# lachinov/brats2019

Hardware: AMD Instinct MI355X
Metric: volumes_per_sec_fwd_bwd_128cubed_x4ch (higher is better)
Workload: dtype bf16

## Files before the change

### brats2019_amd/csrc/pointwise_c16.hip

```cpp
#include "pw_helpers.hpp"
#include "fin_tail.hpp"
#include <type_traits>
#include <stdlib.h>

namespace ru {

typedef float f32x4_c16 __attribute__((ext_vector_type(4)));
template <int I, int N, class F> __device__ __forceinline__ void static_for_c1_impl(F&& f) {
    if constexpr (I < N) { f(std::integral_constant<int, I>{}); static_for_c1_impl<I + 1, N>(f); }
}
template <int N, class F> __device__ __forceinline__ void static_for_c1(F&& f) { static_for_c1_impl<0, N>(f); }

static inline dim3 c16_grid(size_t V, int blocks_nc, unsigned cap = 2048) {
    size_t bx = (V * 4 + 255) / 256;
    if (bx > cap) bx = cap;
    if (bx < 1) bx = 1;
    return dim3((unsigned)bx, (unsigned)blocks_nc);
}

template <int RES, bool NT = false>
__global__ __launch_bounds__(256) void gn_apply16_kernel(const float* __restrict__ x, const float* __restrict__ scale, const float* __restrict__ shift,
                                                         const float* __restrict__ res, float* __restrict__ y, int C, size_t V, float slope,
                                                         const float* __restrict__ rscale, const float* __restrict__ rshift, float rslope) {
    const int nb = blockIdx.y, CB = C >> 4;
// ... 101 lines not shown
    const int nblk = gn_bwd_tiles16(V);
    FinTail f{};
    if (fin) f = *fin;
    RU_REQUIRE(!f.ticket || (f.kind == 2 && f.nblk == nblk && f.N == N && f.C == C && f.G == G), "gn_bwd_reduce16: tail descriptor does not match the launch");
    const size_t lds = 512 + fin_tail_lds_bytes(f);
    RU_REQUIRE(lds <= 64 * 1024, "gn_bwd_reduce16: batch x channels too large for the in-launch finalize");
    hipLaunchKernelGGL(gn_bwd_reduce16_kernel, dim3(nblk, N * (C / 16)), dim3(256), lds, s, x, dy, scale, shift, mean, rstd, slope, partials, C, V, G, nblk, gn16_chunk(V), f);
    RU_CHECK_LAUNCH("gn_bwd_reduce16_kernel");
    return RU_OK;
}

__global__ __launch_bounds__(256) void gn_bwd_apply16_kernel(const float* __restrict__ x, const float* __restrict__ dy, const float* __restrict__ scale,
                                                             const float* __restrict__ shift, const float* __restrict__ coef, float slope,
                                                             float* __restrict__ dx, int C, size_t V) {
    const int nb = blockIdx.y, CB = C >> 4;
    const int n = nb / CB, cb = nb - n * CB;
    const int q = threadIdx.x & 3;
    const size_t row = (size_t)n * C + cb * 16 + 4 * q;
    float a[4], b[4], cA[4], cB[4], cC[4];
#pragma unroll
    for (int k = 0; k < 4; ++k) {
        a[k] = scale[row + k]; b[k] = shift[row + k];
        cA[k] = coef[(row + k) * 3]; cB[k] = coef[(row + k) * 3 + 1]; cC[k] = coef[(row + k) * 3 + 2];
    }
    const size_t base = (size_t)nb * V * 4, F = V * 4;
    const float4* xp = reinterpret_cast<const float4*>(x) + base;
    const float4* dp = reinterpret_cast<const float4*>(dy) + base;
    float4* op = reinterpret_cast<float4*>(dx) + base;
    for (size_t f = (size_t)blockIdx.x * 256 + threadIdx.x; f < F; f += (size_t)gridDim.x * 256) {
        const float4 t = xp[f], d = dp[f];
        float4 o;
        o.x = cA[0] * ((t.x * a[0] + b[0]) > 0.f ? d.x : d.x * slope) + (cB[0] * t.x + cC[0]);
        o.y = cA[1] * ((t.y * a[1] + b[1]) > 0.f ? d.y : d.y * slope) + (cB[1] * t.y + cC[1]);
        o.z = cA[2] * ((t.z * a[2] + b[2]) > 0.f ? d.z : d.z * slope) + (cB[2] * t.z + cC[2]);
        o.w = cA[3] * ((t.w * a[3] + b[3]) > 0.f ? d.w : d.w * slope) + (cB[3] * t.w + cC[3]);
        op[f] = o;
    }
}
__global__ __launch_bounds__(256) void gn_bwd_apply16_split_kernel(const float* __restrict__ x, const float* __restrict__ dy, const float* __restrict__ scale,
                                                                   const float* __restrict__ shift, const float* __restrict__ coef, float slope,
                                                                   float* __restrict__ dx, int C, size_t V) {
    const int nb = blockIdx.y, CB = C >> 4;
    const int n = nb / CB, cb = nb - n * CB;
    const int hf = threadIdx.x & 1;
    const size_t row = (size_t)n * C + cb * 16 + 8 * hf;
    float a[8], b[8], cA[8], cB[8], cC[8];
#pragma unroll
    for (int k = 0; k < 8; ++k) {
        a[k] = scale[row + k]; b[k] = shift[row + k];
        cA[k] = coef[(row + k) * 3]; cB[k] = coef[(row + k) * 3 + 1]; cC[k] = coef[(row + k) * 3 + 2];
    }
    const size_t base = (size_t)nb * V * 4, F = V * 2;
    const float4* xp = reinterpret_cast<const float4*>(x) + base;
    const float4* dp = reinterpret_cast<const float4*>(dy) + base;
    pw_u32x4* op = reinterpret_cast<pw_u32x4*>(dx) + base;
    for (size_t f = (size_t)blockIdx.x * 256 + threadIdx.x; f < F; f += (size_t)gridDim.x * 256) {
        const size_t v = f >> 1;
        const float4 t0 = xp[v * 4 + 2 * hf], t1 = xp[v * 4 + 2 * hf + 1], d0 = dp[v * 4 + 2 * hf], d1 = dp[v * 4 + 2 * hf + 1];
        const float tx[8] = {t0.x, t0.y, t0.z, t0.w, t1.x, t1.y, t1.z, t1.w}, dd[8] = {d0.x, d0.y, d0.z, d0.w, d1.x, d1.y, d1.z, d1.w};
        float o[8];
#pragma unroll
        for (int k = 0; k < 8; ++k) o[k] = cA[k] * ((tx[k] * a[k] + b[k]) > 0.f ? dd[k] : dd[k] * slope) + (cB[k] * tx[k] + cC[k]);
        pw_u32x4 hi, lo;
        pw_split8(o, hi, lo);
        op[v * 4 + hf] = hi;
        op[v * 4 + 2 + hf] = lo;
    }
}
int gn_bwd_apply16_launch(const float* x, const float* dy, const float* scale, const float* shift, const float* coef, float slope, float* dx,
                          int N, int C, size_t V, int split, hipStream_t s) {
    RU_REQUIRE(C % 16 == 0, "gn_bwd_apply16: C must be a multiple of 16");
    if (split) {
        size_t bx = (V * 2 + 255) / 256;
        if (bx > 2048) bx = 2048;
        hipLaunchKernelGGL(gn_bwd_apply16_split_kernel, dim3((unsigned)bx, (unsigned)(N * (C / 16))), dim3(256), 0, s, x, dy, scale, shift, coef, slope, dx, C, V);
    } else {
        hipLaunchKernelGGL(gn_bwd_apply16_kernel, c16_grid(V, N * (C / 16)), dim3(256), 0, s, x, dy, scale, shift, coef, slope, dx, C, V);
    }
    RU_CHECK_LAUNCH("gn_bwd_apply16_kernel");
    return RU_OK;
}

__global__ __launch_bounds__(256) void up2_fwd16_kernel(const float* __restrict__ x, float* __restrict__ y, int D, int H, int W, float slope) {
    const int Do = 2 * D, Ho = 2 * H, Wo = 2 * W;
    const size_t nb = blockIdx.y;
    const size_t Vi = (size_t)D * H * W, Vo = Vi * 8;
    const float4* xp = reinterpret_cast<const float4*>(x) + nb * Vi * 4;
    float4* yp = reinterpret_cast<float4*>(y) + nb * Vo * 4;
    const bool nt_out = (size_t)gridDim.y * Vo * 16 * sizeof(float) >= ((size_t)128 << 20);
    const size_t total = (size_t)(D + 1) * (H + 1) * Wo * 4;
    for (size_t f = (size_t)blockIdx.x * 256 + threadIdx.x; f < total; f += (size_t)gridDim.x * 256) {
        const int q = (int)(f & 3);
        size_t r = f >> 2;
        const int xo = (int)(r % Wo); r /= Wo;
        const int ky = (int)(r % (H + 1)) - 1;
        const int kz = (int)(r / (H + 1)) - 1;
        int x0, x1; float lx0, lx1;
        up2_src(xo, W, x0, x1, lx0, lx1);
        const int zA = kz < 0 ? 0 : kz, zB = kz + 1 > D - 1 ? D - 1 : kz + 1;
        const int yA = ky < 0 ? 0 : ky, yB = ky + 1 > H - 1 ? H - 1 : ky + 1;
        const size_t rAA = ((size_t)zA * H + yA) * W, rAB = ((size_t)zA * H + yB) * W, rBA = ((size_t)zB * H + yA) * W, rBB = ((size_t)zB * H + yB) * W;
        const float4 a00 = xp[(rAA + x0) * 4 + q], b00 = xp[(rAA + x1) * 4 + q];
        const float4 a01 = xp[(rAB + x0) * 4 + q], b01 = xp[(rAB + x1) * 4 + q];
        const float4 a10 = xp[(rBA + x0) * 4 + q], b10 = xp[(rBA + x1) * 4 + q];
        const float4 a11 = xp[(rBB + x0) * 4 + q], b11 = xp[(rBB + x1) * 4 + q];
        float4 e00, e01, e10, e11;
#define RU_UPX(c) e00.c = lx0 * a00.c + lx1 * b00.c; e01.c = lx0 * a01.c + lx1 * b01.c; e10.c = lx0 * a10.c + lx1 * b10.c; e11.c = lx0 * a11.c + lx1 * b11.c
        RU_UPX(x); RU_UPX(y); RU_UPX(z); RU_UPX(w);
#undef RU_UPX
#pragma unroll
        for (int dz = 0; dz < 2; ++dz) {
            const int zo = 2 * kz + 1 + dz;
            if (zo < 0 || zo >= Do) continue;
            int z0, z1; float lz0, lz1;
            up2_src(zo, D, z0, z1, lz0, lz1);
#pragma unroll
            for (int dy = 0; dy < 2; ++dy) {
                const int yo = 2 * ky + 1 + dy;
                if (yo < 0 || yo >= Ho) continue;
                int y0, y1; float ly0, ly1;
                up2_src(yo, H, y0, y1, ly0, ly1);
                float4 o;
#define RU_UP2(c) o.c = lrelu(lz0 * (ly0 * e00.c + ly1 * e01.c) + lz1 * (ly0 * e10.c + ly1 * e11.c), slope)
                RU_UP2(x); RU_UP2(y); RU_UP2(z); RU_UP2(w);
#undef RU_UP2
                if (nt_out) __builtin_nontemporal_store(f32x4_c16{o.x, o.y, o.z, o.w}, reinterpret_cast<f32x4_c16*>(yp + (((size_t)zo * Ho + yo) * Wo + xo) * 4 + q));
                else yp[(((size_t)zo * Ho + yo) * Wo + xo) * 4 + q] = o;
            }
        }
    }
}
int up2_fwd16_launch(const float* x, float* y, int N, int C, int D, int H, int W, float slope, hipStream_t s) {
    RU_REQUIRE(C % 16 == 0, "up2_fwd16: C must be a multiple of 16");
    const size_t total = (size_t)(D + 1) * (H + 1) * (2 * W) * 4;
    size_t bx = (total + 255) / 256;
    if (bx > 16384) bx = 16384;
    hipLaunchKernelGGL(up2_fwd16_kernel, dim3((unsigned)bx, (unsigned)(N * (C / 16))), dim3(256), 0, s, x, y, D, H, W, slope);
    RU_CHECK_LAUNCH("up2_fwd16_kernel");
    return RU_OK;
}

#ifndef RU_UP2B_ZC
#define RU_UP2B_ZC 8
#endif
constexpr int UP2B_ZC = RU_UP2B_ZC;
__global__ __launch_bounds__(256) void up2_bwd16_kernel(const float* __restrict__ dy, float* __restrict__ dx, int D, int H, int W) {
    const int Do = 2 * D, Ho = 2 * H, Wo = 2 * W;
    const size_t nb = blockIdx.y;
    const size_t Vi = (size_t)D * H * W, Vo = Vi * 8;
    const float4* dp = reinterpret_cast<const float4*>(dy) + nb * Vo * 4;
    float4* op = reinterpret_cast<float4*>(dx) + nb * Vi * 4;
    const int nch = (D + UP2B_ZC - 1) / UP2B_ZC;
    const size_t total = (size_t)nch * H * W * 4;
    for (size_t f = (size_t)blockIdx.x * 256 + threadIdx.x; f < total; f += (size_t)gridDim.x * 256) {
        const int q = (int)(f & 3);
        size_t r = f >> 2;
        const int kx = (int)(r % W); r /= W;
        const int ky = (int)(r % H);
        const int k0 = (int)(r / H) * UP2B_ZC;
        const int k1 = k0 + UP2B_ZC < D ? k0 + UP2B_ZC : D;
        float wy[4], wx[4];
        size_t oy[4], ox[4];
#pragma unroll
        for (int t = 0; t < 4; ++t) {
            const int y = 2 * ky - 1 + t, xx = 2 * kx - 1 + t;
            wy[t] = (y >= 0 && y < Ho) ? up2_coef(y, H, ky) : 0.f;
            wx[t] = (xx >= 0 && xx < Wo) ? up2_coef(xx, W, kx) : 0.f;
            oy[t] = (size_t)(y < 0 ? 0 : (y >= Ho ? Ho - 1 : y)) * Wo;
            ox[t] = (size_t)(xx < 0 ? 0 : (xx >= Wo ? Wo - 1 : xx)) * 4 + q;
        }
        float4 accP = make_float4(0.f, 0.f, 0.f, 0.f), accC = accP;
        for (int m = k0; m <= k1; ++m) {
#pragma unroll
            for (int h = 0; h < 2; ++h) {
                const int z = 2 * m - 1 + h;
                const bool in = z >= 0 && z < Do;
                const size_t zrow = (size_t)(z < 0 ? 0 : (z >= Do ? Do - 1 : z)) * Ho * Wo;
                float4 pz = make_float4(0.f, 0.f, 0.f, 0.f);
#pragma unroll
                for (int b = 0; b < 4; ++b) {
                    const float4* row = dp + (zrow + oy[b]) * 4;
                    const float4 p0 = row[ox[0]], p1 = row[ox[1]], p2 = row[ox[2]], p3 = row[ox[3]];
                    pz.x += wy[b] * (wx[0] * p0.x + wx[1] * p1.x + wx[2] * p2.x + wx[3] * p3.x);
                    pz.y += wy[b] * (wx[0] * p0.y + wx[1] * p1.y + wx[2] * p2.y + wx[3] * p3.y);
                    pz.z += wy[b] * (wx[0] * p0.z + wx[1] * p1.z + wx[2] * p2.z + wx[3] * p3.z);
                    pz.w += wy[b] * (wx[0] * p0.w + wx[1] * p1.w + wx[2] * p2.w + wx[3] * p3.w);
                }
                const float cP = (in && m - 1 >= k0) ? up2_coef(z, D, m - 1) : 0.f;
                const float cC = (in && m < k1) ? up2_coef(z, D, m) : 0.f;
                accP.x += cP * pz.x; accP.y += cP * pz.y; accP.z += cP * pz.z; accP.w += cP * pz.w;
                accC.x += cC * pz.x; accC.y += cC * pz.y; accC.z += cC * pz.z; accC.w += cC * pz.w;
            }
            if (m - 1 >= k0) op[(((size_t)(m - 1) * H + ky) * W + kx) * 4 + q] = accP;
            accP = accC;
            accC = make_float4(0.f, 0.f, 0.f, 0.f);
        }
    }
}
int up2_bwd16_launch(const float* dy, float* dx, int N, int C, int D, int H, int W, hipStream_t s) {
    RU_REQUIRE(C % 16 == 0, "up2_bwd16: C must be a multiple of 16");
    const size_t total = (size_t)((D + UP2B_ZC - 1) / UP2B_ZC) * H * W * 4;
    size_t bx = (total + 255) / 256;
    if (bx > 16384) bx = 16384;
    hipLaunchKernelGGL(up2_bwd16_kernel, dim3((unsigned)bx, (unsigned)(N * (C / 16))), dim3(256), 0, s, dy, dx, D, H, W);
    RU_CHECK_LAUNCH("up2_bwd16_kernel");
    return RU_OK;
}

__global__ void pack_down16_kernel(const float* __restrict__ w, float* __restrict__ wd, float* __restrict__ wdT, int Cout, int Cin) {
    const int i = blockIdx.x * blockDim.x + threadIdx.x;
    if (i >= Cout * Cin * 8) return;
    const int tap = i & 7, c = (i >> 3) % Cin, o = i / (8 * Cin);
    const float v = w[i];
    wd[(size_t)o * 8 * Cin + tap * Cin + c] = v;
    wdT[(size_t)(tap * Cin + c) * Cout + o] = v;
}
int pack_down16_launch(const float* w, float* wd, float* wdT, int Cout, int Cin, hipStream_t s) {
    const int total = Cout * Cin * 8;
    hipLaunchKernelGGL(pack_down16_kernel, dim3(cdiv(total, 256)), dim3(256), 0, s, w, wd, wdT, Cout, Cin);
    RU_CHECK_LAUNCH("pack_down16_kernel");
    return RU_OK;
}

template <int COB, int S2D, int NSLOT, bool PAIR = false>
__global__ __launch_bounds__(256, (PAIR || NSLOT > 0) ? 2 : 1) void conv1_16_kernel(const Conv1Args a, int nvt) {
    static_assert(!PAIR || (S2D == 2 && COB == 4 && (NSLOT == 1 || NSLOT == 2)), "paired stores: the scatter mode with statistics, four blocks per workgroup");
    constexpr bool BST = NSLOT > 0;
    constexpr int NSL = BST ? NSLOT : 1;
    __shared__ float red[BST ? 4 * NSL * 16 * 2 : 1];
    const int lane = threadIdx.x & 63, wave = threadIdx.x >> 6;
    const int n = blockIdx.z, cog = blockIdx.y;
    const size_t V = a.V;
    const int r = lane & 15, g = lane >> 4;
    const int nkb0 = a.C0 >> 4, nkb1 = a.C1 >> 4, nkb = nkb0 + nkb1, CBo = a.Cout >> 4;
    const int Hf = 2 * a.Hc, Wf = 2 * a.Wc;
    const size_t Vf = V * 8;
    const int CBf_out = CBo >> 3;
    const int Cstat = S2D == 2 ? (a.Cout >> 3) : a.Cout;
    f32x4_c16 bs1[NSL], bs2[NSL], bk[NSL][3];
    if constexpr (BST) {
#pragma unroll
        for (int sl = 0; sl < NSL; ++sl) {
            bs1[sl] = f32x4_c16{0.f, 0.f, 0.f, 0.f}; bs2[sl] = f32x4_c16{0.f, 0.f, 0.f, 0.f};
            const int cob = cog * COB + sl, chb = S2D == 2 ? cob % CBf_out : cob;
            const float* kp = a.bst_k + (size_t)n * 3 * Cstat + (cob < CBo ? chb : 0) * 16 + 4 * g;
#pragma unroll
            for (int t3 = 0; t3 < 3; ++t3) { const float4 q = *reinterpret_cast<const float4*>(kp + (size_t)t3 * Cstat); bk[sl][t3] = f32x4_c16{q.x, q.y, q.z, q.w}; }
        }
    }
    const bool nt_out = (size_t)a.N * a.Cout * V * sizeof(float) >= ((size_t)128 << 20);
    const int vt = blockIdx.x * 4 + wave;
    const bool live = vt < nvt;
    if (!live) { if constexpr (!BST) return; }
    if (live) {
    const size_t v0 = (size_t)vt * 64;
    size_t vb[4], fv[4];
#pragma unroll
    for (int t = 0; t < 4; ++t) {
        size_t v = v0 + 16 * t + r;
        if (v >= V) v = V - 1;
        vb[t] = v * 16 + 4 * g;
        fv[t] = 0;
        if constexpr (S2D != 0) {
            const int xc = (int)(v % a.Wc);
            const size_t rr = v / a.Wc;
            const int yc = (int)(rr % a.Hc), zc = (int)(rr / a.Hc);
            fv[t] = ((size_t)(2 * zc) * Hf + 2 * yc) * Wf + 2 * xc;
        }
    }
    const float* wrow[COB];
#pragma unroll
    for (int cb = 0; cb < COB; ++cb) {
        const int cob = cog * COB + cb;
        wrow[cb] = a.wT + (size_t)((cob < CBo ? cob : CBo - 1) * 16 + r) * a.ldw + 4 * g;
    }
    f32x4_c16 acc[4][COB];
#pragma unroll
    for (int t = 0; t < 4; ++t)
#pragma unroll
        for (int cb = 0; cb < COB; ++cb) acc[t][cb] = f32x4_c16{0.f, 0.f, 0.f, 0.f};
    const int CBf_in = nkb0 >> 3;
    auto kstep = [&](int kb) __attribute__((always_inline)) {
        float4 xb[4];
        if constexpr (S2D == 1) {
            const int tap = kb / CBf_in, cbf = kb - tap * CBf_in;
            const size_t toff = ((size_t)(tap >> 2) * Hf + ((tap >> 1) & 1)) * Wf + (tap & 1);
            const float* src = a.x0 + ((size_t)(n * CBf_in + cbf) * Vf) * 16 + 4 * g;
#pragma unroll
            for (int t = 0; t < 4; ++t) xb[t] = *reinterpret_cast<const float4*>(src + (fv[t] + toff) * 16);
        } else {
            const float* src = kb < nkb0 ? a.x0 + ((size_t)(n * nkb0 + kb) * V) * 16 : a.x1 + ((size_t)(n * nkb1 + kb - nkb0) * V) * 16;
#pragma unroll
            for (int t = 0; t < 4; ++t) xb[t] = *reinterpret_cast<const float4*>(src + vb[t]);
        }
#pragma unroll
        for (int cb = 0; cb < COB; ++cb) {
            const float4 wv = *reinterpret_cast<const float4*>(wrow[cb] + kb * 16);
#pragma unroll
            for (int t = 0; t < 4; ++t) {
                acc[t][cb] = __builtin_amdgcn_mfma_f32_16x16x4f32(wv.x, xb[t].x, acc[t][cb], 0, 0, 0);
                acc[t][cb] = __builtin_amdgcn_mfma_f32_16x16x4f32(wv.y, xb[t].y, acc[t][cb], 0, 0, 0);
                acc[t][cb] = __builtin_amdgcn_mfma_f32_16x16x4f32(wv.z, xb[t].z, acc[t][cb], 0, 0, 0);
                acc[t][cb] = __builtin_amdgcn_mfma_f32_16x16x4f32(wv.w, xb[t].w, acc[t][cb], 0, 0, 0);
            }
        }
    };
    int kb = 0;
// ... 290 lines not shown
```

### brats2019_amd/csrc/wgrad_tr.hip

```cpp
#include "ru_common.h"

#include <utility>

namespace ru {

typedef float f32x4 __attribute__((ext_vector_type(4)));
typedef __bf16 bf16x8 __attribute__((ext_vector_type(8)));
typedef __bf16 bf16x2 __attribute__((ext_vector_type(2)));
typedef short s16x4 __attribute__((ext_vector_type(4)));
typedef short s16x8 __attribute__((ext_vector_type(8)));
typedef unsigned int u32x4 __attribute__((ext_vector_type(4)));


template <int... Is, class F>
__device__ __forceinline__ void wt_static_for_impl(std::integer_sequence<int, Is...>, F&& f) {
    (f(std::integral_constant<int, Is>{}), ...);
}
template <int N, class F>
__device__ __forceinline__ void wt_static_for(F&& f) {
    wt_static_for_impl(std::make_integer_sequence<int, N>{}, static_cast<F&&>(f));
}

__device__ __forceinline__ void wt_split8(const float (&t)[8], u32x4& hi, u32x4& lo) {
    split_n<4>(t, hi, lo);
}

__device__ __forceinline__ void wt_hi8(const float (&t)[8], u32x4& hi) {
#pragma unroll
    for (int i = 0; i < 4; ++i) {
        ru_bf16x2 h;
        h[0] = (__bf16)t[2 * i];
        h[1] = (__bf16)t[2 * i + 1];
        hi[i] = __builtin_bit_cast(unsigned, h);
    }
}

__device__ __forceinline__ bf16x8 wt_read_tr(const char* p0, const char* p1) {
    const s16x4 a = __builtin_amdgcn_ds_read_tr16_b64_v4i16((s16x4 __attribute__((address_space(3)))*)(p0));
    const s16x4 b = __builtin_amdgcn_ds_read_tr16_b64_v4i16((s16x4 __attribute__((address_space(3)))*)(p1));
    const s16x8 r = {a[0], a[1], a[2], a[3], b[0], b[1], b[2], b[3]};
    return __builtin_bit_cast(bf16x8, r);
}

template <int OT>
struct WTZ {
    static constexpr int TY = 8, HY = 10, HX = 18, NSLOT = 8;
    static constexpr int PPOS = HY * HX;
    static constexpr int PLANE = PPOS * 32;
    static constexpr int XRING = NSLOT * PLANE;
    static constexpr int X_OFF = 0, XLO_OFF = XRING;
    static constexpr int DPOS = 2 * TY * 16, DPLANE = DPOS * 32;
    static constexpr int DBUF = OT * 2 * DPLANE;
    static constexpr int D_OFF = 2 * XRING;
    static constexpr int LDS = 2 * XRING + 2 * DBUF;
    static constexpr int NKB = 8;
};

template <int OT, int NP, bool PACK>
__device__ __forceinline__ void wtz_consume(const char* __restrict__ xl, const int (&pw)[3], const char* __restrict__ dl, f32x4 (&acc)[27]) {
    using P = WTZ<OT>;
    constexpr int HX = P::HX, NHALF = OT, NG = PACK ? 3 : 9, NU = NHALF * NG;
    bf16x8 bh[2][4], bl[2][4];
    bf16x8 ah[2][2], al[2][2];
    auto read_one = [&](auto U, auto R) {
        constexpr int u = decltype(U)::value, r = NP == 3 ? decltype(R)::value : 2 * decltype(R)::value;
        constexpr int h = u / NG, g = u % NG, dz = PACK ? g : g / 3, dx = PACK ? 0 : g % 3, set = u & 1;
        if constexpr (r < 8) {
            constexpr int pr = r >> 1;
            constexpr int off0 = ((4 * h + pr) * HX + dx) * 32, off1 = off0 + 2 * HX * 32;
            const char* p = xl + pw[dz];
            if constexpr ((r & 1) == 0) bh[set][pr] = wt_read_tr(p + P::X_OFF + off0, p + P::X_OFF + off1);
            else bl[set][pr] = wt_read_tr(p + P::XLO_OFF + off0, p + P::XLO_OFF + off1);
        } else {
            constexpr int ra = r - 8, kbi = ra >> 1;
            constexpr int off0 = (4 * h + kbi) * 16 * 32, off1 = off0 + 2 * 16 * 32;
            if constexpr ((ra & 1) == 0) ah[h & 1][kbi] = wt_read_tr(dl + off0, dl + off1);
            else al[h & 1][kbi] = wt_read_tr(dl + P::DPLANE + off0, dl + P::DPLANE + off1);
        }
    };
    auto nreads = [](int u) constexpr { return ((u % NG == 0) ? 12 : 8) / (NP == 3 ? 1 : 2); };
    wt_static_for<nreads(0)>([&](auto R) { read_one(std::integral_constant<int, 0>{}, R); });
    wt_static_for<NU>([&](auto U) {
        constexpr int u = decltype(U)::value, h = u / NG, g = u % NG, dz = PACK ? g : g / 3, dx = PACK ? 0 : g % 3, set = u & 1;
        constexpr int nr = u + 1 < NU ? nreads(u + 1) : 0;
        constexpr int NM = 6 * NP;
        wt_static_for<NM>([&](auto M) {
            constexpr int m = decltype(M)::value, prod = NP == 3 ? m / 6 : 2, kbi = (m / 3) % 2, dy = m % 3;
            constexpr int tap = PACK ? dz * 3 + dy : dz * 9 + dy * 3 + dx, pr = kbi + dy;
            if constexpr (prod == 0) acc[tap] = __builtin_amdgcn_mfma_f32_16x16x32_bf16(al[h & 1][kbi], bh[set][pr], acc[tap], 0, 0, 0);
            if constexpr (prod == 1) acc[tap] = __builtin_amdgcn_mfma_f32_16x16x32_bf16(ah[h & 1][kbi], bl[set][pr], acc[tap], 0, 0, 0);
            if constexpr (prod == 2) acc[tap] = __builtin_amdgcn_mfma_f32_16x16x32_bf16(ah[h & 1][kbi], bh[set][pr], acc[tap], 0, 0, 0);
            __builtin_amdgcn_sched_barrier(0);
            constexpr int ra = m * nr / NM, rb = (m + 1) * nr / NM;
            wt_static_for<rb - ra>([&](auto K) {
                read_one(std::integral_constant<int, u + 1>{}, std::integral_constant<int, ra + decltype(K)::value>{});
            });
            __builtin_amdgcn_sched_barrier(0);
        });
    });
}

template <int OT, int XS, int DS, int NP = 3>
__global__ __launch_bounds__(512, 2) void wgrad3_tz_kernel(const Wgrad3Args a, float* __restrict__ partials, int ntz, int nty, int ntx, int ncg, int CoP, int CiP) {
    using P = WTZ<OT>;
    constexpr int HX = P::HX, PPOS = P::PPOS, DPOS = P::DPOS, TY = P::TY;
    constexpr bool FA = DS == 3 || DS == 4, G16 = DS == 4;
    extern __shared__ __attribute__((aligned(256))) char lds[];

    const int tid = threadIdx.x, lane = tid & 63;
    const int wave = __builtin_amdgcn_readfirstlane(tid >> 6);
    const bool producer = wave >= 4;
    const int rw = wave & 3, ptid = tid & 255;
    const int og = blockIdx.y / ncg, cgp = blockIdx.y % ncg;
    const int D = a.D, H = a.H, W = a.W;
    const size_t DHW = (size_t)D * H * W;
    const int CBi = a.Cin >> 4, CBo = a.Cout >> 4;
    const int cols_per_sample = nty * ntx, ncol = a.N * cols_per_sample;
    const int G = gridDim.x;
    const int swz = (G % 8 == 0) ? (blockIdx.x % 8) * (G / 8) + blockIdx.x / 8 : blockIdx.x;
    const int mycols = swz < ncol ? (ncol - swz + G - 1) / G : 0;
    const int nitems = mycols * ntz;
    const int colstride = 2 * ntz + 2;
    const bool xform = a.in_scale != nullptr;
    const float slope = xform ? a.in_slope : 1.f;

    auto item_origin = [&](int item, int& n, int& k, int& y0, int& x0, int& ring0) {
        const int j = item / ntz;
        k = item - j * ntz;
        int b = swz + j * G;
        n = b / cols_per_sample;
        b -= n * cols_per_sample;
        const int tx = b % ntx, ty = b / ntx;
        y0 = ty * TY; x0 = tx * 16;
        ring0 = j * colstride;
    };

    if (producer) {
        if constexpr (G16) __builtin_amdgcn_s_setreg(1 | (23 << 6), 1);
        constexpr int NRX = (4 * PPOS + 127) / 128, NR2 = (2 * PPOS + 127) / 128, NRD = OT * ((DPOS + 127) / 128);
        const int hsel = ptid & 1, pslot = ptid >> 1;
        float4 vx[NRX][2], vd[NRD][2];
        float4 vg[FA ? NRD : 1][2], gc4[FA ? 10 : 1];
        int st_n = 0, st_y0 = 0, st_x0 = 0;
        float4 sc4[2], sh4[2];
        unsigned mx = 0, md = 0, mx2 = 0;
        int stx_ring0 = 0, stx_k = 0, std_k = 0;
        int nx_n = 0, nx_k = 0, nx_y0 = 0, nx_x0 = 0;
        int is_k = 0, is_n = 0, is_y0 = 0, is_x0 = 0, is_ring0 = 0;
        auto load_gc = [&](int n, int q) __attribute__((always_inline)) {
            if constexpr (FA) {
                const size_t go = (size_t)n * a.Cout + (og * OT + q) * 16 + hsel * 8;
                gc4[0] = *reinterpret_cast<const float4*>(a.gb_scale + go); gc4[1] = *reinterpret_cast<const float4*>(a.gb_scale + go + 4);
                gc4[2] = *reinterpret_cast<const float4*>(a.gb_shift + go); gc4[3] = *reinterpret_cast<const float4*>(a.gb_shift + go + 4);
#pragma unroll
                for (int t = 0; t < 6; ++t) gc4[4 + t] = *reinterpret_cast<const float4*>(a.gb_coef + go * 3 + 4 * t);
            }
        };
        auto issue_x = [&](int item) {
            if (item < nitems) {
                if (is_k == 0) item_origin(item, is_n, is_k, is_y0, is_x0, is_ring0);
                nx_n = is_n; nx_k = is_k; nx_y0 = is_y0; nx_x0 = is_x0;
                stx_ring0 = is_ring0; stx_k = is_k;
                if (++is_k == ntz) is_k = 0;
            }
            const int n = nx_n, k = nx_k, y0 = nx_y0, x0 = nx_x0;
            const int hp0 = k == 0 ? 0 : 2 * k + 2, npl = k == 0 ? 4 : 2;
            const float* xb = a.x + ((size_t)(n * CBi + cgp) * DHW) * 16 + hsel * 8;
            mx = 0; mx2 = 0;
            auto xround = [&](auto R) {
                constexpr int r = decltype(R)::value;
                const int u = r * 128 + pslot;
                const int pl = u / PPOS, p = u - pl * PPOS;
                const int hy = p / HX, xc = p - hy * HX;
                const int gz = hp0 + pl - 1, gy = y0 + hy - 1, gx = x0 + xc - 1;
                const bool live = pl < npl;
                const bool ok = live && (unsigned)gz < (unsigned)D && (unsigned)gy < (unsigned)H && (unsigned)gx < (unsigned)W;
#if defined(RU_SB2_DBG) && (RU_SB2_DBG & (1 << 24))
                const size_t ofs = 0;
#else
                const size_t ofs = ok ? (size_t)((gz * H + gy) * W + gx) * 16 : 0;
#endif
                if constexpr (XS == 1) {
                    mx |= (ok && hsel == 0) ? (1u << r) : 0u;
                    vx[r][0] = *reinterpret_cast<const float4*>(a.x + (size_t)n * DHW * 4 + (ofs >> 2));
                    vx[r][1] = make_float4(0.f, 0.f, 0.f, 0.f);
                } else if constexpr (XS == 2) {
                    const bool rowok = live && (unsigned)gz < (unsigned)D && (unsigned)gy < (unsigned)H;
                    const int g0 = gx + 2 * hsel, g1 = g0 + 1;
                    const bool ok0 = rowok && (unsigned)g0 < (unsigned)W, ok1 = rowok && (unsigned)g1 < (unsigned)W;
                    mx |= ok0 ? (1u << r) : 0u;
                    mx2 |= ok1 ? (1u << r) : 0u;
                    const float* x4 = a.x + (size_t)n * DHW * 4;
                    const size_t row = rowok ? (size_t)(gz * H + gy) * W : 0;
                    vx[r][0] = *reinterpret_cast<const float4*>(x4 + (row + (ok0 ? g0 : 0)) * 4);
                    vx[r][1] = *reinterpret_cast<const float4*>(x4 + (row + (ok1 ? g1 : 0)) * 4);
                } else {
                    mx |= ok ? (1u << r) : 0u;
                    vx[r][0] = *reinterpret_cast<const float4*>(xb + ofs);
                    vx[r][1] = *reinterpret_cast<const float4*>(xb + ofs + 4);
                }
            };
            wt_static_for<NR2>(xround);
            if (k == 0) wt_static_for<NRX - NR2>([&](auto R) { xround(std::integral_constant<int, NR2 + decltype(R)::value>{}); });
            if (xform) {
                const int cofs = n * a.Cin + cgp * 16 + hsel * 8;
                sc4[0] = *reinterpret_cast<const float4*>(a.in_scale + cofs); sc4[1] = *reinterpret_cast<const float4*>(a.in_scale + cofs + 4);
                sh4[0] = *reinterpret_cast<const float4*>(a.in_shift + cofs); sh4[1] = *reinterpret_cast<const float4*>(a.in_shift + cofs + 4);
            }
        };
        auto issue_d = [&]() {
            const int n = nx_n, k = nx_k, y0 = nx_y0, x0 = nx_x0;
            std_k = k;
            md = 0;
#pragma unroll
            for (int r = 0; r < NRD; ++r) {
                constexpr int RPB = (DPOS + 127) / 128;
                const int q = r / RPB, p = (r - q * RPB) * 128 + pslot;
                const int row = p >> 4, xc = p & 15;
                const int z = row / TY, y = row - z * TY;
                const int gz = 2 * k + z, gy = y0 + y, gx = x0 + xc;
                const bool ok = p < DPOS && gz < D && gy < H && gx < W;
                const float* db = a.dy + ((size_t)(n * CBo + og * OT + q) * DHW) * 16 + hsel * 8;
#if defined(RU_SB2_DBG) && (RU_SB2_DBG & (1 << 24))
                const size_t ofs = 0;
#else
                const size_t ofs = ok ? (size_t)((gz * H + gy) * W + gx) * 16 : 0;
#endif
                if constexpr (FA) {
                    md |= ok ? (1u << r) : 0u;
                    const size_t cb = ((size_t)(n * CBo + og * OT + q) * DHW) * 16 + ofs + hsel * 8;
                    vd[r][0] = *reinterpret_cast<const float4*>(a.gb_y + cb);
                    vd[r][1] = *reinterpret_cast<const float4*>(a.gb_y + cb + 4);
                    vg[r][0] = *reinterpret_cast<const float4*>(a.gb_d + cb);
                    vg[r][1] = *reinterpret_cast<const float4*>(a.gb_d + cb + 4);
                } else if constexpr (DS == 1) {
                    md |= ok ? (1u << r) : 0u;
                    const float* ds = a.dy + ((size_t)(n * CBo + og * OT + q) * DHW) * 16 + ofs + hsel * 4;
                    vd[r][0] = *reinterpret_cast<const float4*>(ds);
                    if constexpr (NP == 3) vd[r][1] = *reinterpret_cast<const float4*>(ds + 8);
                } else if constexpr (DS == 2) {
                    md |= (ok && hsel == 0) ? (1u << r) : 0u;
                    vd[r][0] = *reinterpret_cast<const float4*>(a.dy + (size_t)n * DHW * 4 + (ofs >> 2));
                    vd[r][1] = make_float4(0.f, 0.f, 0.f, 0.f);
                } else {
                    md |= ok ? (1u << r) : 0u;
                    vd[r][0] = *reinterpret_cast<const float4*>(db + ofs);
                    vd[r][1] = *reinterpret_cast<const float4*>(db + ofs + 4);
                }
            }
            if constexpr (FA) {
                if constexpr (OT == 1) load_gc(n, 0);
                st_n = n; st_y0 = y0; st_x0 = x0;
            }
        };
        auto store_x = [&]() {
            float sc[8] = {1.f, 1.f, 1.f, 1.f, 1.f, 1.f, 1.f, 1.f}, sh[8] = {0.f, 0.f, 0.f, 0.f, 0.f, 0.f, 0.f, 0.f};
            if (xform) {
                sc[0] = sc4[0].x; sc[1] = sc4[0].y; sc[2] = sc4[0].z; sc[3] = sc4[0].w; sc[4] = sc4[1].x; sc[5] = sc4[1].y; sc[6] = sc4[1].z; sc[7] = sc4[1].w;
                sh[0] = sh4[0].x; sh[1] = sh4[0].y; sh[2] = sh4[0].z; sh[3] = sh4[0].w; sh[4] = sh4[1].x; sh[5] = sh4[1].y; sh[6] = sh4[1].z; sh[7] = sh4[1].w;
            }
            const int hp0 = stx_k == 0 ? 0 : 2 * stx_k + 2, npl = stx_k == 0 ? 4 : 2;
            auto xbody = [&](auto XFORM) {
                constexpr bool XF = decltype(XFORM)::value;
            auto sround = [&](auto R) {
                constexpr int r = decltype(R)::value;
                const int u = r * 128 + pslot;
                const int pl = u / PPOS, p = u - pl * PPOS;
                if (pl >= npl) return;
                const bool ok = (mx >> r) & 1u;
                const bool ok_hi = XS == 2 ? ((mx2 >> r) & 1u) != 0 : ok;
                const float f[8] = {vx[r][0].x, vx[r][0].y, vx[r][0].z, vx[r][0].w, vx[r][1].x, vx[r][1].y, vx[r][1].z, vx[r][1].w};
                float t[8];
#pragma unroll
                for (int c = 0; c < 8; ++c) {
                    const bool okc = c < 4 ? ok : ok_hi;
                    if constexpr (XF) {
                        const float u2 = fmaf(f[c], sc[c], sh[c]);
                        t[c] = okc ? fmaxf(u2, u2 * slope) : 0.f;
                    } else {
                        t[c] = okc ? f[c] : 0.f;
                    }
                }
                u32x4 hi, lo;
                if constexpr (NP == 3) wt_split8(t, hi, lo);
                else wt_hi8(t, hi);
                const int slot = (stx_ring0 + hp0 + pl) & (P::NSLOT - 1);
                char* dst = lds + slot * P::PLANE + p * 32 + hsel * 16;
                *reinterpret_cast<u32x4*>(dst + P::X_OFF) = hi;
                if constexpr (NP == 3) *reinterpret_cast<u32x4*>(dst + P::XLO_OFF) = lo;
            };
            wt_static_for<NR2>(sround);
            if (stx_k == 0) wt_static_for<NRX - NR2>([&](auto R) { sround(std::integral_constant<int, NR2 + decltype(R)::value>{}); });
            };
            if (xform) xbody(std::true_type{});
            else xbody(std::false_type{});
        };
        auto store_d = [&](char* dbuf) {
#pragma unroll
            for (int r = 0; r < NRD; ++r) {
                constexpr int RPB = (DPOS + 127) / 128;
                const int q = r / RPB, p = (r - q * RPB) * 128 + pslot;
                if constexpr (FA && OT > 1) {
                    if (r % RPB == 0) load_gc(st_n, q);
                }
                const bool ok = (md >> r) & 1u;
                const float f[8] = {vd[r][0].x, vd[r][0].y, vd[r][0].z, vd[r][0].w, vd[r][1].x, vd[r][1].y, vd[r][1].z, vd[r][1].w};
                float t[8];
                if constexpr (FA) {
                    const float g[8] = {vg[r][0].x, vg[r][0].y, vg[r][0].z, vg[r][0].w, vg[r][1].x, vg[r][1].y, vg[r][1].z, vg[r][1].w};
                    const float ga[8] = {gc4[0].x, gc4[0].y, gc4[0].z, gc4[0].w, gc4[1].x, gc4[1].y, gc4[1].z, gc4[1].w};
                    const float gb[8] = {gc4[2].x, gc4[2].y, gc4[2].z, gc4[2].w, gc4[3].x, gc4[3].y, gc4[3].z, gc4[3].w};
                    const float cf[24] = {gc4[4].x, gc4[4].y, gc4[4].z, gc4[4].w, gc4[5].x, gc4[5].y, gc4[5].z, gc4[5].w, gc4[6].x, gc4[6].y, gc4[6].z, gc4[6].w,
                                          gc4[7].x, gc4[7].y, gc4[7].z, gc4[7].w, gc4[8].x, gc4[8].y, gc4[8].z, gc4[8].w, gc4[9].x, gc4[9].y, gc4[9].z, gc4[9].w};
#pragma unroll
                    for (int c = 0; c < 8; ++c) {
                        const float dyv = cf[3 * c] * ((f[c] * ga[c] + gb[c]) > 0.f ? g[c] : g[c] * a.gb_slope) + (cf[3 * c + 1] * f[c] + cf[3 * c + 2]);
                        t[c] = ok ? dyv : 0.f;
                    }
                } else {
#pragma unroll
                    for (int c = 0; c < 8; ++c) t[c] = ok ? f[c] : 0.f;
                }
                u32x4 hi, lo = u32x4{0u, 0u, 0u, 0u};
                float lof[FA ? 8 : 1], amax = 0.f;
                if constexpr (DS == 1) {
                    const u32x4 z = u32x4{0u, 0u, 0u, 0u};
                    hi = ok ? __builtin_bit_cast(u32x4, vd[r][0]) : z;
                    if constexpr (NP == 3) lo = ok ? __builtin_bit_cast(u32x4, vd[r][1]) : z;
                } else if constexpr (FA) {
                    amax = mxg_hi8(t, hi, lof);
#pragma unroll
                    for (int c = 0; c < 4; ++c) {
                        ru_bf16x2 l2;
                        l2[0] = (__bf16)lof[2 * c]; l2[1] = (__bf16)lof[2 * c + 1];
                        lo[c] = __builtin_bit_cast(unsigned, l2);
                    }
                } else if constexpr (NP == 3) {
                    wt_split8(t, hi, lo);
                } else {
                    wt_hi8(t, hi);
                }
                *reinterpret_cast<u32x4*>(dbuf + q * 2 * P::DPLANE + p * 32 + hsel * 16) = hi;
                if constexpr (NP == 3) *reinterpret_cast<u32x4*>(dbuf + q * 2 * P::DPLANE + P::DPLANE + p * 32 + hsel * 16) = lo;
                if constexpr (FA) {
                    if (ok && cgp == 0 && a.gb_out) {
                        const int row = p >> 4, z = row / TY;
                        const size_t vox = (size_t)((2 * std_k + z) * H + st_y0 + (row - z * TY)) * W + st_x0 + (p & 15);
                        u32x4* op = reinterpret_cast<u32x4*>(a.gb_out) + ((size_t)(st_n * CBo + og * OT + q) * DHW + vox) * 4;
                        op[hsel] = hi;
                        if constexpr (G16) {
                            const float m = fmaxf(amax, __builtin_bit_cast(float, __builtin_amdgcn_update_dpp(0, __builtin_bit_cast(int, amax), 0xb1, 0xf, 0xf, true)));
                            unsigned l8[2], x8[2];
                            mxg_cvt8(t, lof, m, l8, x8);
                            op[2 + hsel] = u32x4{l8[0], l8[1], x8[0], x8[1]};
                        } else {
                            op[2 + hsel] = lo;
                        }
                    }
                }
            }
        };
        if (nitems > 0) {
            issue_x(0);
            issue_d();
            store_x();
            issue_x(1);
            store_d(lds + P::D_OFF);
            issue_d();
        }
        __syncthreads();
        for (int w = 0; w < nitems; ++w) {
            if (w + 1 < nitems) {
                store_x();
                issue_x(w + 2);
                store_d(lds + P::D_OFF + ((w + 1) & 1) * P::DBUF);
                issue_d();
            }
            __syncthreads();
        }
        __syncthreads();
    } else {
        f32x4 acc[27];
#pragma unroll
        for (int t = 0; t < 27; ++t) acc[t] = f32x4{0.f, 0.f, 0.f, 0.f};
        const int i16 = lane & 15, g = lane >> 4;
        const int lane_off = (4 * g + (i16 >> 2)) * 32 + (i16 & 3) * 8;
        const int zw = rw >> 1;
        const int yb = OT == 1 ? 4 * (rw & 1) : 0, qw = OT == 1 ? 0 : (rw & 1);
        const int xrow_off = yb * HX * 32 + lane_off;
        const int drow_off = (zw * TY + yb) * 16 * 32 + qw * 2 * P::DPLANE + lane_off;
        __syncthreads();
        int cj = 0, ck = 0;
        for (int w = 0; w < nitems; ++w) {
            const int j = cj, k = ck;
            if (++ck == ntz) { ck = 0; ++cj; }
            const int s0 = j * colstride + 2 * k + zw;
            int pw[3];
#pragma unroll
            for (int p = 0; p < 3; ++p) pw[p] = ((s0 + p) & (P::NSLOT - 1)) * P::PLANE + xrow_off;
            const char* dl = lds + P::D_OFF + (w & 1) * P::DBUF + drow_off;
            wtz_consume<OT, NP, XS == 2>(lds, pw, dl, acc);
            __syncthreads();
        }
        f32x4* red = reinterpret_cast<f32x4*>(lds);
        constexpr int NT = XS == 2 ? 9 : 27;
#pragma unroll
        for (int t = 0; t < NT; ++t) red[(rw * 27 + t) * 64 + lane] = acc[t];
        __syncthreads();
    }
    {
        const f32x4* red = reinterpret_cast<const f32x4*>(lds);
        const int c0 = cgp * 16;
        constexpr int NT = XS == 2 ? 9 : 27;
        for (int e = tid; e < OT * NT * 64; e += 512) {
            const int q = e & 63, t = (e >> 6) % NT, ot = (e >> 6) / NT;
            f32x4 v;
            if constexpr (OT == 1) v = (red[(0 * 27 + t) * 64 + q] + red[(1 * 27 + t) * 64 + q]) + (red[(2 * 27 + t) * 64 + q] + red[(3 * 27 + t) * 64 + q]);
            else v = red[(ot * 27 + t) * 64 + q] + red[((ot + 2) * 27 + t) * 64 + q];
            int c = c0 + (q & 15), tap = t;
            bool live = true;
            if constexpr (XS == 2) {
                const int j = (q & 15) >> 2;
                c = q & 3;
                tap = (t / 3) * 9 + (t % 3) * 3 + j;
                live = j < 3;
            }
#pragma unroll
            for (int r = 0; r < 4; ++r) {
                const int o = og * OT * 16 + ot * 16 + (q >> 4) * 4 + r;
                if (live && o < CoP && c < CiP) partials[(((size_t)blockIdx.x * 27 + tap) * CoP + o) * CiP + c] = v[r];
            }
        }
    }
}

struct WTRChoice { int ot, nbx, ngroups, ncg; };
static WTRChoice wtr_choose(int N, int Cin, int Cout, int D, int H, int W) {
    WTRChoice c;
    c.ot = (Cout >= 32 && (Cout / 16) % 2 == 0) ? 2 : 1;
    c.ncg = Cin / 16;
    c.ngroups = (Cout / 16 / c.ot) * c.ncg;
    const long ntile = (long)N * cdiv(D, 4) * cdiv(H, 4) * cdiv(W, 16);
    long nbx = 256 / c.ngroups;
    if (nbx < 1) nbx = 1;
    if (nbx > ntile) nbx = ntile;
    c.nbx = (int)nbx;
    return c;
}

size_t wgrad3_tr_workspace_bytes(int N, int Cin, int Cout, int D, int H, int W) {
    if (Cin % 16 || Cout % 16) return 0;
    const WTRChoice c = wtr_choose(N, Cin, Cout, D, H, W);
    return (size_t)c.nbx * 27 * Cout * Cin * sizeof(float);
}

enum { WTR_NO_LAYOUT = -1, WTR_NO_GB_OPERANDS = -2, WTR_NO_G16 = -3, WTR_NO_C4_GB = -4, WTR_NO_C4_OT2 = -5, WTR_NO_C4_BLOCK = -6, WTR_NO_TWO_C4 = -7, WTR_NO_C4_XFORM = -8 };
static constexpr int wtr_pack(int ot, int xs, int ds, int np = 3) { return ot | (xs << 4) | (ds << 8) | (np << 12); }
int wgrad3_tr_inst(const Wgrad3Args& a) {
    if (!(a.x_c16 && a.dy_c16 && a.Cin > 0 && a.Cout > 0 && a.Cin % 16 == 0 && a.Cout % 16 == 0)) return WTR_NO_LAYOUT;
    const int ot = wtr_choose(a.N, a.Cin, a.Cout, a.D, a.H, a.W).ot;
    const bool p1 = a.products == 1;
    if (a.x_c4 && a.in_scale) return WTR_NO_C4_XFORM;
    if (a.gb_y) {
        if (!(!a.dy_c4 && a.gb_d && a.gb_scale && a.gb_shift && a.gb_coef && (a.gb_out || a.x_c4))) return WTR_NO_GB_OPERANDS;
        const bool g16 = a.gb_g16 != 0;
        if (g16 && !(ot == 1 && !p1 && !a.x_c4)) return WTR_NO_G16;
        if (a.x_c4) {
            if (!(ot == 1 && a.Cin == 16)) return WTR_NO_C4_GB;
            return wtr_pack(1, 2, 3, p1 ? 1 : 3);
        }
        if (ot == 2) return wtr_pack(2, 0, 3);
        if (p1) return wtr_pack(1, 0, 3, 1);
        return wtr_pack(1, 0, g16 ? 4 : 3);
    }
    const int xs = a.x_c4 ? 1 : 0, ds = a.dy_c4 ? 2 : (a.dy_s16 ? 1 : 0);
    if (ot == 2) {
        if (!(xs == 0 && ds != 2)) return WTR_NO_C4_OT2;
        return wtr_pack(2, 0, ds, (p1 && ds == 1) ? 1 : 3);
    }
    if (!((xs == 0 || a.Cin == 16) && (ds != 2 || a.Cout == 16))) return WTR_NO_C4_BLOCK;
    if (xs == 1) {
        if (ds == 2) return WTR_NO_TWO_C4;
        if (ds == 1) return wtr_pack(1, 2, 1);
        return wtr_pack(1, 2, 0, p1 ? 1 : 3);
    }
    if (ds == 2) return wtr_pack(1, 0, 2, p1 ? 1 : 3);
    return wtr_pack(1, 0, ds);
}

template <int OT, int XS, int DS, int NP = 3>
static int wtz_cfg(const Wgrad3Args& a, const WTRChoice& c, hipStream_t s) {
    using P = WTZ<OT>;
    static PerDevice attr_done;
    if (!attr_done.get()) {
        hipError_t e = hipFuncSetAttribute(reinterpret_cast<const void*>(wgrad3_tz_kernel<OT, XS, DS, NP>), hipFuncAttributeMaxDynamicSharedMemorySize, P::LDS);
        if (e != hipSuccess) return hip_fail(e, "hipFuncSetAttribute(wgrad3_tz)");
        attr_done.set();
    }
    const int ntz = cdiv(a.D, 2), nty = cdiv(a.H, 8), ntx = cdiv(a.W, 16);
    const long ncol = (long)a.N * nty * ntx;
    int nbx = c.nbx;
    if (nbx > ncol) nbx = (int)ncol;
    hipLaunchKernelGGL((wgrad3_tz_kernel<OT, XS, DS, NP>), dim3(nbx, c.ngroups), dim3(512), P::LDS, s, a, (float*)a.ws, ntz, nty, ntx, c.ncg, a.Cout, a.Cin);
    RU_CHECK_LAUNCH("wgrad3_tz_kernel");
    const int co = a.dw_cout > 0 ? a.dw_cout : a.Cout, ci = a.dw_cin > 0 ? a.dw_cin : a.Cin;
    if (a.swapped) return wgrad_reduce_launch((const float*)a.ws, nbx, 27, a.Cout, a.Cin, co, ci, a.dw, 27, co * 27, 0, s, 1, a.defer);
    return wgrad_reduce_launch((const float*)a.ws, nbx, 27, a.Cout, a.Cin, co, ci, a.dw, ci * 27, 27, 0, s, 0, a.defer);
}

int wgrad3_tr_launch(const Wgrad3Args& a, hipStream_t s) {
    const int inst = wgrad3_tr_inst(a);
    RU_REQUIRE(inst != WTR_NO_LAYOUT, "wgrad3_tr: needs voxel-major x and dy with channel counts %% 16 == 0");
    const WTRChoice c = wtr_choose(a.N, a.Cin, a.Cout, a.D, a.H, a.W);
    if (!a.ws || a.ws_bytes < wgrad3_tr_workspace_bytes(a.N, a.Cin, a.Cout, a.D, a.H, a.W)) {
        set_error("wgrad3_tr: workspace too small");
        return RU_ENOMEM;
    }
    RU_REQUIRE(inst != WTR_NO_C4_XFORM, "wgrad3_tr: a 4-channel copy of x takes no fused transform");
    RU_REQUIRE(inst != WTR_NO_GB_OPERANDS, "wgrad3_tr: the fused GroupNorm-backward apply needs all of its operands");
    RU_REQUIRE(inst != WTR_NO_G16, "wgrad3_tr: the gradient-operand form is published by the one-block, three-product kernel on a voxel-major x only");
    RU_REQUIRE(inst != WTR_NO_C4_GB, "wgrad3_tr: a 4-channel copy stands for ONE 16-channel block");
    RU_REQUIRE(inst != WTR_NO_C4_OT2 && inst != WTR_NO_C4_BLOCK, "wgrad3_tr: 4-channel copies stand for ONE 16-channel block");
    RU_REQUIRE(inst != WTR_NO_TWO_C4, "wgrad3_tr: only one operand can be a 4-channel copy");
    switch (inst) {
        case wtr_pack(1, 2, 3, 1): return wtz_cfg<1, 2, 3, 1>(a, c, s);
        case wtr_pack(1, 2, 3): return wtz_cfg<1, 2, 3>(a, c, s);
        case wtr_pack(1, 0, 3, 1): return wtz_cfg<1, 0, 3, 1>(a, c, s);
        case wtr_pack(2, 0, 3): return wtz_cfg<2, 0, 3>(a, c, s);
        case wtr_pack(1, 0, 4): return wtz_cfg<1, 0, 4>(a, c, s);
        case wtr_pack(1, 0, 3): return wtz_cfg<1, 0, 3>(a, c, s);
        case wtr_pack(2, 0, 1, 1): return wtz_cfg<2, 0, 1, 1>(a, c, s);
        case wtr_pack(2, 0, 1): return wtz_cfg<2, 0, 1>(a, c, s);
        case wtr_pack(2, 0, 0): return wtz_cfg<2, 0, 0>(a, c, s);
        case wtr_pack(1, 2, 1): return wtz_cfg<1, 2, 1>(a, c, s);
        case wtr_pack(1, 2, 0, 1): return wtz_cfg<1, 2, 0, 1>(a, c, s);
        case wtr_pack(1, 2, 0): return wtz_cfg<1, 2, 0>(a, c, s);
        case wtr_pack(1, 0, 2, 1): return wtz_cfg<1, 0, 2, 1>(a, c, s);
        case wtr_pack(1, 0, 2): return wtz_cfg<1, 0, 2>(a, c, s);
        case wtr_pack(1, 0, 1): return wtz_cfg<1, 0, 1>(a, c, s);
        case wtr_pack(1, 0, 0): return wtz_cfg<1, 0, 0>(a, c, s);
    }
    set_error("wgrad3_tr: no kernel for instantiation %d", inst);
    return RU_EINVAL;
}

}
```

Measured before the change: 270.6.

## Double producer waves for 4-channel wgrad and swizzle upsample-backward blocks

For the 4-channel (XS==2) weight-gradient kernel, the block grows from 8 to 12 waves so eight producer waves load and stage x and dy. Each producer thread now handles one x position and writes it to both halves of the overlapping LDS row layout, which removes the hsel half-split. The fused input transform is disabled for that path, and debug bits guarded by a macro can skip stages. Separately, upsample backward remaps block indices with an 8-way swizzle like the wgrad kernel; the larger blocks risk lower occupancy and more register pressure.

```diff
diff --git a/brats2019_amd/csrc/pointwise_c16.hip b/brats2019_amd/csrc/pointwise_c16.hip
--- a/brats2019_amd/csrc/pointwise_c16.hip
+++ b/brats2019_amd/csrc/pointwise_c16.hip
@@ -277,7 +277,9 @@
     float4* op = reinterpret_cast<float4*>(dx) + nb * Vi * 4;
     const int nch = (D + UP2B_ZC - 1) / UP2B_ZC;
     const size_t total = (size_t)nch * H * W * 4;
-    for (size_t f = (size_t)blockIdx.x * 256 + threadIdx.x; f < total; f += (size_t)gridDim.x * 256) {
+    const unsigned G = gridDim.x;
+    const unsigned swz = (G % 8 == 0) ? (blockIdx.x % 8) * (G / 8) + blockIdx.x / 8 : blockIdx.x;
+    for (size_t f = (size_t)swz * 256 + threadIdx.x; f < total; f += (size_t)G * 256) {
         const int q = (int)(f & 3);
         size_t r = f >> 2;
         const int kx = (int)(r % W); r /= W;
diff --git a/brats2019_amd/csrc/wgrad_tr.hip b/brats2019_amd/csrc/wgrad_tr.hip
--- a/brats2019_amd/csrc/wgrad_tr.hip
+++ b/brats2019_amd/csrc/wgrad_tr.hip
@@ -100,17 +100,26 @@
     });
 }
 
+#ifdef RU_SB2_DBG
+constexpr int kWtzDbg = RU_SB2_DBG;
+#else
+constexpr int kWtzDbg = 0;
+#endif
+template <int XS> constexpr int WTZ_NPROD = (XS == 2 && !(kWtzDbg & (1 << 28))) ? 8 : 4;
+template <int XS> constexpr int WTZ_NTHR = 64 * (4 + WTZ_NPROD<XS>);
 template <int OT, int XS, int DS, int NP = 3>
-__global__ __launch_bounds__(512, 2) void wgrad3_tz_kernel(const Wgrad3Args a, float* __restrict__ partials, int ntz, int nty, int ntx, int ncg, int CoP, int CiP) {
+__global__ __launch_bounds__(WTZ_NTHR<XS>, (WTZ_NTHR<XS> / 256)) void wgrad3_tz_kernel(const Wgrad3Args a, float* __restrict__ partials, int ntz, int nty, int ntx, int ncg, int CoP, int CiP) {
     using P = WTZ<OT>;
     constexpr int HX = P::HX, PPOS = P::PPOS, DPOS = P::DPOS, TY = P::TY;
+    constexpr int NTHR = WTZ_NTHR<XS>, RS = WTZ_NPROD<XS> * 32;
+    static_assert(DPOS % RS == 0, "a dy round has no dead positions: store_d writes every p it computes");
     constexpr bool FA = DS == 3 || DS == 4, G16 = DS == 4;
     extern __shared__ __attribute__((aligned(256))) char lds[];
 
     const int tid = threadIdx.x, lane = tid & 63;
     const int wave = __builtin_amdgcn_readfirstlane(tid >> 6);
     const bool producer = wave >= 4;
-    const int rw = wave & 3, ptid = tid & 255;
+    const int rw = wave & 3, ptid = tid - 256;
     const int og = blockIdx.y / ncg, cgp = blockIdx.y % ncg;
     const int D = a.D, H = a.H, W = a.W;
     const size_t DHW = (size_t)D * H * W;
@@ -121,7 +130,7 @@
     const int mycols = swz < ncol ? (ncol - swz + G - 1) / G : 0;
     const int nitems = mycols * ntz;
     const int colstride = 2 * ntz + 2;
-    const bool xform = a.in_scale != nullptr;
+    const bool xform = XS != 2 && a.in_scale != nullptr;
     const float slope = xform ? a.in_slope : 1.f;
 
     auto item_origin = [&](int item, int& n, int& k, int& y0, int& x0, int& ring0) {
@@ -137,7 +146,8 @@
 
     if (producer) {
         if constexpr (G16) __builtin_amdgcn_s_setreg(1 | (23 << 6), 1);
-        constexpr int NRX = (4 * PPOS + 127) / 128, NR2 = (2 * PPOS + 127) / 128, NRD = OT * ((DPOS + 127) / 128);
+        constexpr int XPP = XS == 2 ? P::HY * (HX + 2) : PPOS, XU = XS == 2 ? 2 * RS : RS;
+        constexpr int NRX = (4 * XPP + XU - 1) / XU, NR2 = (2 * XPP + XU - 1) / XU, NRD = OT * (DPOS / RS);
         const int hsel = ptid & 1, pslot = ptid >> 1;
         float4 vx[NRX][2], vd[NRD][2];
         float4 vg[FA ? NRD : 1][2], gc4[FA ? 10 : 1];
@@ -169,9 +179,10 @@
             mx = 0; mx2 = 0;
             auto xround = [&](auto R) {
                 constexpr int r = decltype(R)::value;
-                const int u = r * 128 + pslot;
-                const int pl = u / PPOS, p = u - pl * PPOS;
-                const int hy = p / HX, xc = p - hy * HX;
+                constexpr int RW = XS == 2 ? HX + 2 : HX;
+                const int u = r * XU + (XS == 2 ? ptid : pslot);
+                const int pl = u / XPP, p = u - pl * XPP;
+                const int hy = p / RW, xc = p - hy * RW;
                 const int gz = hp0 + pl - 1, gy = y0 + hy - 1, gx = x0 + xc - 1;
                 const bool live = pl < npl;
                 const bool ok = live && (unsigned)gz < (unsigned)D && (unsigned)gy < (unsigned)H && (unsigned)gx < (unsigned)W;
@@ -186,7 +197,7 @@
                     vx[r][1] = make_float4(0.f, 0.f, 0.f, 0.f);
                 } else if constexpr (XS == 2) {
                     const bool rowok = live && (unsigned)gz < (unsigned)D && (unsigned)gy < (unsigned)H;
-                    const int g0 = gx + 2 * hsel, g1 = g0 + 1;
+                    const int g0 = gx, g1 = g0 + 1;
                     const bool ok0 = rowok && (unsigned)g0 < (unsigned)W, ok1 = rowok && (unsigned)g1 < (unsigned)W;
                     mx |= ok0 ? (1u << r) : 0u;
                     mx2 |= ok1 ? (1u << r) : 0u;
@@ -214,8 +225,8 @@
             md = 0;
 #pragma unroll
             for (int r = 0; r < NRD; ++r) {
-                constexpr int RPB = (DPOS + 127) / 128;
-                const int q = r / RPB, p = (r - q * RPB) * 128 + pslot;
+                constexpr int RPB = DPOS / RS;
+                const int q = r / RPB, p = (r - q * RPB) * RS + pslot;
                 const int row = p >> 4, xc = p & 15;
                 const int z = row / TY, y = row - z * TY;
                 const int gz = 2 * k + z, gy = y0 + y, gx = x0 + xc;
@@ -264,8 +275,8 @@
                 constexpr bool XF = decltype(XFORM)::value;
             auto sround = [&](auto R) {
                 constexpr int r = decltype(R)::value;
-                const int u = r * 128 + pslot;
-                const int pl = u / PPOS, p = u - pl * PPOS;
+                const int u = r * XU + (XS == 2 ? ptid : pslot);
+                const int pl = u / XPP, p = u - pl * XPP;
                 if (pl >= npl) return;
                 const bool ok = (mx >> r) & 1u;
                 const bool ok_hi = XS == 2 ? ((mx2 >> r) & 1u) != 0 : ok;
@@ -285,9 +296,22 @@
                 if constexpr (NP == 3) wt_split8(t, hi, lo);
                 else wt_hi8(t, hi);
                 const int slot = (stx_ring0 + hp0 + pl) & (P::NSLOT - 1);
-                char* dst = lds + slot * P::PLANE + p * 32 + hsel * 16;
-                *reinterpret_cast<u32x4*>(dst + P::X_OFF) = hi;
-                if constexpr (NP == 3) *reinterpret_cast<u32x4*>(dst + P::XLO_OFF) = lo;
+                if constexpr (XS == 2) {
+                    const int hy = p / (HX + 2), s = p - hy * (HX + 2);
+                    char* dst = lds + slot * P::PLANE + (hy * HX + s) * 32;
+                    if (s < HX) {
+                        *reinterpret_cast<u32x4*>(dst + P::X_OFF) = hi;
+                        if constexpr (NP == 3) *reinterpret_cast<u32x4*>(dst + P::XLO_OFF) = lo;
+                    }
+                    if (s >= 2) {
+                        *reinterpret_cast<u32x4*>(dst + P::X_OFF - 48) = hi;
+                        if constexpr (NP == 3) *reinterpret_cast<u32x4*>(dst + P::XLO_OFF - 48) = lo;
+                    }
+                } else {
+                    char* dst = lds + slot * P::PLANE + p * 32 + hsel * 16;
+                    *reinterpret_cast<u32x4*>(dst + P::X_OFF) = hi;
+                    if constexpr (NP == 3) *reinterpret_cast<u32x4*>(dst + P::XLO_OFF) = lo;
+                }
             };
             wt_static_for<NR2>(sround);
             if (stx_k == 0) wt_static_for<NRX - NR2>([&](auto R) { sround(std::integral_constant<int, NR2 + decltype(R)::value>{}); });
@@ -298,8 +322,8 @@
         auto store_d = [&](char* dbuf) {
 #pragma unroll
             for (int r = 0; r < NRD; ++r) {
-                constexpr int RPB = (DPOS + 127) / 128;
-                const int q = r / RPB, p = (r - q * RPB) * 128 + pslot;
+                constexpr int RPB = DPOS / RS;
+                const int q = r / RPB, p = (r - q * RPB) * RS + pslot;
                 if constexpr (FA && OT > 1) {
                     if (r % RPB == 0) load_gc(st_n, q);
                 }
@@ -360,7 +384,7 @@
                 }
             }
         };
-        if (nitems > 0) {
+        if (nitems > 0 && !(kWtzDbg & (1 << 30))) {
             issue_x(0);
             issue_d();
             store_x();
@@ -370,7 +394,7 @@
         }
         __syncthreads();
         for (int w = 0; w < nitems; ++w) {
-            if (w + 1 < nitems) {
+            if (w + 1 < nitems && !(kWtzDbg & (1 << 30))) {
                 store_x();
                 issue_x(w + 2);
                 store_d(lds + P::D_OFF + ((w + 1) & 1) * P::DBUF);
@@ -399,7 +423,7 @@
 #pragma unroll
             for (int p = 0; p < 3; ++p) pw[p] = ((s0 + p) & (P::NSLOT - 1)) * P::PLANE + xrow_off;
             const char* dl = lds + P::D_OFF + (w & 1) * P::DBUF + drow_off;
-            wtz_consume<OT, NP, XS == 2>(lds, pw, dl, acc);
+            if constexpr (!(kWtzDbg & (1 << 29))) wtz_consume<OT, NP, XS == 2>(lds, pw, dl, acc);
             __syncthreads();
         }
         f32x4* red = reinterpret_cast<f32x4*>(lds);
@@ -412,7 +436,7 @@
         const f32x4* red = reinterpret_cast<const f32x4*>(lds);
         const int c0 = cgp * 16;
         constexpr int NT = XS == 2 ? 9 : 27;
-        for (int e = tid; e < OT * NT * 64; e += 512) {
+        for (int e = tid; e < OT * NT * 64; e += NTHR) {
             const int q = e & 63, t = (e >> 6) % NT, ot = (e >> 6) / NT;
             f32x4 v;
             if constexpr (OT == 1) v = (red[(0 * 27 + t) * 64 + q] + red[(1 * 27 + t) * 64 + q]) + (red[(2 * 27 + t) * 64 + q] + red[(3 * 27 + t) * 64 + q]);
@@ -501,7 +525,7 @@
     const long ncol = (long)a.N * nty * ntx;
     int nbx = c.nbx;
     if (nbx > ncol) nbx = (int)ncol;
-    hipLaunchKernelGGL((wgrad3_tz_kernel<OT, XS, DS, NP>), dim3(nbx, c.ngroups), dim3(512), P::LDS, s, a, (float*)a.ws, ntz, nty, ntx, c.ncg, a.Cout, a.Cin);
+    hipLaunchKernelGGL((wgrad3_tz_kernel<OT, XS, DS, NP>), dim3(nbx, c.ngroups), dim3(WTZ_NTHR<XS>), P::LDS, s, a, (float*)a.ws, ntz, nty, ntx, c.ncg, a.Cout, a.Cin);
     RU_CHECK_LAUNCH("wgrad3_tz_kernel");
     const int co = a.dw_cout > 0 ? a.dw_cout : a.Cout, ci = a.dw_cin > 0 ? a.dw_cin : a.Cin;
     if (a.swapped) return wgrad_reduce_launch((const float*)a.ws, nbx, 27, a.Cout, a.Cin, co, ci, a.dw, 27, co * 27, 0, s, 1, a.defer);
```

Result: no change. 271.4 (median of 6 runs) (+0.3%).
